# spcl/gemm_hls

Hardware: NVIDIA H100
Metric: GFLOP/s at N=16384 K=16384 M=16384 float (Multiply,Add) (higher is better)
Workload: dtype tf32 tensor-core multiply, f32 accumulate/storage

## Files before the change

gemm_hls_b200/csrc/gemm_tcgen05.cu:

```cuda
#include <cuda.h>
#include <cuda_fp16.h>
#include <cuda_runtime.h>

#include <algorithm>
#include <cstdlib>
#include <cstring>
#include <vector>

#include "common.cuh"
#include "fits_half.h"
#include "gemm_wgmma.cuh"
#include "ptx_sm90.cuh"
#include "tma_host.cuh"

namespace mm {
namespace {

__device__ __forceinline__ float round_tf32(float x) {
  uint32_t r;
  asm("cvt.rna.tf32.f32 %0, %1;" : "=r"(r) : "f"(x));
  const bool overflowed = (r & 0x7FFFFFFFu) == 0x7F800000u && (__float_as_uint(x) & 0x7FFFFFFFu) != 0x7F800000u;
  return __uint_as_float(overflowed ? ((r & 0x80000000u) | 0x7F7FE000u) : r);
}

// ... 14 lines not shown
    v.y = round_tf32(v.y);
    v.z = round_tf32(v.z);
    v.w = round_tf32(v.w);
    dst[i] = v;
  }
}

constexpr int FP_TILE = 64;
constexpr int FP_THREADS = 256;

struct FloatPrepOperand {
  const float *src = nullptr;
  float *dst = nullptr;
  __half *dst16 = nullptr;
  unsigned int *fits = nullptr;
  const unsigned int *partner = nullptr;
  uint32_t partner_stride = 0;
  const unsigned int *other = nullptr;
  uint32_t other_count = 0;
  unsigned char *pending = nullptr;
  uint32_t src_rows = 0, src_cols = 0, tiles_c = 0, items_per_copy = 0, items = 0;
  bool transpose = false;
  bool vec = false;
};
struct FloatPrepArgs {
  FloatPrepOperand op[2];
};

struct FloatItemSmem {
  float tile[FP_TILE][FP_TILE + 1];
  int settled;
};

__device__ __forceinline__ bool settled_now(const FloatPrepOperand &o, uint32_t copy) {
  const volatile unsigned int *own = o.fits;
  if (own[copy] == 0u) return true;
  const volatile unsigned int *partner = o.partner;
  return partner != nullptr && partner[copy * o.partner_stride] == 0u;
}

template <bool COMPLETE>
__device__ __forceinline__ void float_item(const FloatPrepOperand &o, uint32_t item, FloatItemSmem &sm) {
  const uint32_t t = threadIdx.x;
  const uint32_t copy = item / o.items_per_copy;
  const uint32_t tile_i = item - copy * o.items_per_copy;
  const uint32_t r0 = tile_i / o.tiles_c * FP_TILE, c0 = tile_i % o.tiles_c * FP_TILE;
  const size_t base = size_t(copy) * o.src_rows * o.src_cols;
  const float *src = o.src + base;
  float v[16];
  bool fit = true;
  if (!o.transpose) {
#pragma unroll
    for (int j = 0; j < 2; ++j) {
      const uint32_t q = t + FP_THREADS * j, r = r0 + q / 8, c = c0 + 8 * (q % 8);
      float4 x = make_float4(0.f, 0.f, 0.f, 0.f), y = x;
      if (r < o.src_rows && c < o.src_cols) {
        const float4 *p = reinterpret_cast<const float4 *>(src + size_t(r) * o.src_cols + c);
        x = p[0];
        y = p[1];
      }
      v[8 * j + 0] = x.x; v[8 * j + 1] = x.y; v[8 * j + 2] = x.z; v[8 * j + 3] = x.w;
      v[8 * j + 4] = y.x; v[8 * j + 5] = y.y; v[8 * j + 6] = y.z; v[8 * j + 7] = y.w;
    }
  } else {
#pragma unroll
    for (int j = 0; j < 4; ++j) {
      const uint32_t f = t + FP_THREADS * j, r = r0 + f / 16, c = c0 + 4 * (f % 16);
      float4 x = make_float4(0.f, 0.f, 0.f, 0.f);
      if (r < o.src_rows) {
        const float *p = src + size_t(r) * o.src_cols + c;
        if (o.vec) {
          if (c < o.src_cols) x = *reinterpret_cast<const float4 *>(p);
        } else {
          if (c + 0 < o.src_cols) x.x = p[0];
          if (c + 1 < o.src_cols) x.y = p[1];
          if (c + 2 < o.src_cols) x.z = p[2];
          if (c + 3 < o.src_cols) x.w = p[3];
        }
      }
      v[4 * j + 0] = x.x; v[4 * j + 1] = x.y; v[4 * j + 2] = x.z; v[4 * j + 3] = x.w;
    }
  }
#pragma unroll
  for (int e = 0; e < 16; ++e) {
    v[e] = round_tf32(v[e]);
    if (!COMPLETE) fit = fit && tf32_fits_half(__float_as_uint(v[e]));
  }
  if (o.transpose) {
#pragma unroll
    for (int j = 0; j < 4; ++j) {
      const uint32_t f = t + FP_THREADS * j, r = f / 16, c = 4 * (f % 16);
#pragma unroll
      for (int e = 0; e < 4; ++e) sm.tile[r][c + e] = v[4 * j + e];
    }
  }
  if (!COMPLETE && t == 0) sm.settled = settled_now(o, copy);
  __syncthreads();
  const bool settled = COMPLETE || sm.settled;
  float *dst = o.dst + base;
  __half *dst16 = o.dst16 + base;
  const uint32_t ld = o.transpose ? o.src_rows : o.src_cols;
  if (!o.transpose) {
#pragma unroll
    for (int j = 0; j < 2; ++j) {
      const uint32_t q = t + FP_THREADS * j, r = r0 + q / 8, c = c0 + 8 * (q % 8);
      if (r >= o.src_rows || c >= o.src_cols) continue;
      const size_t off = size_t(r) * ld + c;
      const float *w = v + 8 * j;
      if (settled) {
        reinterpret_cast<float4 *>(dst + off)[0] = make_float4(w[0], w[1], w[2], w[3]);
        reinterpret_cast<float4 *>(dst + off)[1] = make_float4(w[4], w[5], w[6], w[7]);
      } else {
        *reinterpret_cast<uint4 *>(dst16 + off) =
            make_uint4(half2_bits(w[0], w[1]), half2_bits(w[2], w[3]), half2_bits(w[4], w[5]), half2_bits(w[6], w[7]));
      }
    }
  } else if (settled) {
#pragma unroll
    for (int j = 0; j < 4; ++j) {
      const uint32_t idx = t + FP_THREADS * j, m = idx % 4 + 4 * (idx / 64), g = idx / 4 % 16;
      if (c0 + m >= o.src_cols || r0 + 4 * g >= o.src_rows) continue;
      float4 x;
      x.x = sm.tile[4 * g + 0][m];
      x.y = sm.tile[4 * g + 1][m];
      x.z = sm.tile[4 * g + 2][m];
      x.w = sm.tile[4 * g + 3][m];
      *reinterpret_cast<float4 *>(dst + size_t(c0 + m) * ld + r0 + 4 * g) = x;
    }
  } else {
#pragma unroll
// ... 436 lines not shown

int float_prep_grid(const void *kernel, uint32_t items) {
  MM_CUDA_TRY(cudaFuncSetAttribute(kernel, cudaFuncAttributePreferredSharedMemoryCarveout,
                                   cudaSharedmemCarveoutMaxShared));
  int per_sm = 0;
  MM_CUDA_TRY(cudaOccupancyMaxActiveBlocksPerMultiprocessor(&per_sm, kernel, FP_THREADS, 0));
  return int(std::max<uint32_t>(1u, std::min<uint32_t>(items, uint32_t(std::max(per_sm, 1) * num_sms()))));
}
}

int tcgen05_prepare_float(bool complete, const void *a, unsigned row0, unsigned rows, const void *b, unsigned n,
                          unsigned k, unsigned m, int flags, const Tuning &t, const GemmBatch &batch, void *scratch,
                          size_t scratch_bytes, cudaStream_t stream) {
  const HalfScratch hs = tcgen05_half_scratch(scratch, scratch_bytes, MM_DTYPE_FLOAT, n, k, m, flags, t, batch);
  if (hs.fits_a == nullptr) return fail(MM_ERR_INVALID, "tcgen05_prepare_float: float on the default datapath only");
  if (row0 % FP_TILE != 0) return fail(MM_ERR_INVALID, "tcgen05_prepare_float: A's first row must be a multiple of 64");
  unsigned char *sp = static_cast<unsigned char *>(scratch);
  const bool shared_a = batch.count > 1 && batch.shared_a, shared_b = batch.count > 1 && batch.shared_b;
  FloatPrepArgs args;
  if (b != nullptr) {
    FloatPrepOperand &o = args.op[0];
    o = float_operand(b, reinterpret_cast<float *>(sp), static_cast<__half *>(hs.b), k, m, batch.b_copies(), true,
                      hs.fits_b, hs.pending_b);
    o.partner = shared_b ? nullptr : hs.fits_a;
    o.partner_stride = shared_a ? 0 : 1;
    o.other = hs.fits_a;
    o.other_count = batch.a_copies();
  }
  if (a != nullptr) {
    const bool transposed = (flags & MM_FLAG_TRANSPOSED_A) != 0;
    if (transposed && (row0 != 0 || rows != n)) return fail(MM_ERR_INVALID, "A stored K x N is prepared whole");
    const size_t first = size_t(row0) * k;
    float *aprep = reinterpret_cast<float *>(sp + tcgen05_bt_bytes(MM_DTYPE_FLOAT, k, m, flags, t, batch.b_copies()));
    FloatPrepOperand &o = args.op[1];
    o = float_operand(a, aprep + first, static_cast<__half *>(hs.a) + first, transposed ? k : rows,
                      transposed ? rows : k, batch.a_copies(), transposed, hs.fits_a,
                      hs.pending_a + size_t(row0 / FP_TILE) * ceil_div(k, FP_TILE));
    o.partner = shared_a ? nullptr : hs.fits_b;
    o.partner_stride = shared_b ? 0 : 1;
    o.other = hs.fits_b;
    o.other_count = batch.b_copies();
  }
  const uint32_t items = args.op[0].items + args.op[1].items;
  if (complete) {
    const int grid = float_prep_grid(reinterpret_cast<const void *>(complete_tf32_kernel), items);
    complete_tf32_kernel<<<grid, FP_THREADS, 0, stream>>>(args);
// ... 135 lines not shown
```

gemm_hls_b200/csrc/gemm_wgmma.cuh:

```cuda
#pragma once

#include <cuda.h>
#include <cuda_bf16.h>
#include <cuda_fp16.h>
#include <cuda_runtime.h>

#include <algorithm>
#include <cstring>
#include <type_traits>

#include "common.cuh"
#include "ptx_sm90.cuh"
#include "tma_host.cuh"

namespace mm {
namespace {

constexpr int BLOCK_M = 128;
constexpr int BLOCK_K_BYTES = 128;
constexpr int WGMMA_K_BYTES = 32;
constexpr int NUM_THREADS = 384;
constexpr int CONSUMER_WARPS = 8;
constexpr int EPI_ROWS = 16;
constexpr int EPI_BUF_BYTES = 2048;
constexpr int EPI_BYTES = CONSUMER_WARPS * EPI_BUF_BYTES;
constexpr int BAR_BYTES = 256;
constexpr int MAX_DYN_SMEM = 232448;

template <int CG, int BN>
struct Geo {
  static constexpr int LOAD_N = BN / CG;
  static constexpr int A_STAGE_BYTES = BLOCK_M * BLOCK_K_BYTES;
  static constexpr int B_STAGE_BYTES = BN * BLOCK_K_BYTES;
  static constexpr int STAGE_BYTES = A_STAGE_BYTES + B_STAGE_BYTES;
  static constexpr int FIT = (MAX_DYN_SMEM - 1024 - BAR_BYTES - EPI_BYTES) / STAGE_BYTES;
  static constexpr int MAX_STAGES = FIT < 8 ? FIT : 8;
  static constexpr int TILE_ROWS = BLOCK_M * CG;
  static constexpr size_t smem_bytes(int stages) {
    return size_t(stages) * STAGE_BYTES + EPI_BYTES + 1024  + BAR_BYTES;
  }
};

struct TileCoord {
  uint32_t r, c;
  uint32_t prob;
};

__device__ __forceinline__ TileCoord tile_coord(uint32_t t, uint32_t tiles_r, uint32_t tiles_c,
// ... 179 lines not shown
        const int32_t a_row = tc.prob * p.a_prob_rows + tc.r * G::TILE_ROWS + cta_rank * BLOCK_M;
        const int32_t b_row = tc.prob * p.b_prob_rows + tc.c * BN + cta_rank * G::LOAD_N;
        if (p.b_ready != nullptr && int32_t(tc.c) != ready_panel) {
          const unsigned int *flag = p.b_ready + tc.c;
          const long long t0 = clock64();
          while (ld_acquire_gpu(flag) < p.b_ready_target) {
            if (clock64() - t0 > (1ll << 34)) __trap();
          }
          asm volatile("fence.proxy.async.global;" ::: "memory");
          ready_panel = int32_t(tc.c);
        }
        const bool h = half_tile(tc);
        const CUtensorMap *map_a = h ? &tmap_a16 : &tmap_a;
        const CUtensorMap *map_b = h ? &tmap_b16 : &tmap_b;
        const uint32_t tile_kb = h ? num_kb16 : num_kb;
        const int32_t kb_elems = h ? BLOCK_K_BYTES / 2 : BLOCK_K_ELEMS;
        for (uint32_t kb = 0; kb < tile_kb; ++kb) {
          ptx::mbar_wait(empty_bar(stage), phase ^ 1);
          const uint32_t sa = smem_a0 + stage * G::A_STAGE_BYTES;
          const uint32_t sb = smem_b0 + stage * G::B_STAGE_BYTES + cta_rank * G::LOAD_N * BLOCK_K_BYTES;
          const int32_t k0 = kb * kb_elems;
          ptx::mbar_arrive_expect_tx(full_bar(stage), G::STAGE_BYTES);
          ptx::tma_load_2d(sa, map_a, full_bar(stage), k0, a_row, p.l2_policy);
          if (CG == 1) {
            ptx::tma_load_2d(sb, map_b, full_bar(stage), k0, b_row, p.l2_policy);
          } else {
            ptx::tma_load_2d_multicast(sb, map_b, full_bar(stage), k0, b_row, 0x3, p.l2_policy);
          }
          if (++stage == STAGES) { stage = 0; phase ^= 1; }
        }
        if (p.tile_sync != nullptr && cta_rank == 0) atomicAdd(p.tile_sync, 1u);
      }
    }
  } else {
    ptx::setmaxnreg_inc<232>();
    const uint32_t wg = warp / 4 - 1;
    const uint32_t cwarp = warp - 4;
    const uint32_t buf = epi0 + cwarp * EPI_BUF_BYTES;
    const uint32_t peer = cta_rank ^ 1u;
    uint32_t stage = 0, phase = 0;
    uint32_t acc[BN / 2];
    for (uint32_t t = group_id; t < num_tiles; t += num_groups) {
      const TileCoord tc = tile_coord(t, tiles_r, tiles_c, p.raster_group);
      auto mainloop = [&](auto kind, uint32_t tile_kb) {
        uint32_t prev = 0;
        for (uint32_t kb = 0; kb < tile_kb; ++kb) {
          ptx::mbar_wait(full_bar(stage), phase);
          const uint64_t adesc = ptx::make_smem_desc_k_sw128(smem_a0 + stage * G::A_STAGE_BYTES + wg * 64 * BLOCK_K_BYTES);
          const uint64_t bdesc = ptx::make_smem_desc_k_sw128(smem_b0 + stage * G::B_STAGE_BYTES);
          ptx::wgmma_fence();
#pragma unroll
          for (int k = 0; k < BLOCK_K_BYTES / WGMMA_K_BYTES; ++k) {
            ptx::wgmma<decltype(kind)::value, BN>(acc, adesc + uint64_t(k * (WGMMA_K_BYTES >> 4)),
                                                  bdesc + uint64_t(k * (WGMMA_K_BYTES >> 4)),
                                                  (kb | uint32_t(k)) != 0u ? 1u : 0u);
          }
          ptx::wgmma_commit();
          ptx::wgmma_wait<1>();
          if (kb > 0 && lane == 0) {
            ptx::mbar_arrive(empty_bar(prev));
            if (CG == 2) ptx::mbar_arrive_cluster(empty_bar(prev), peer);
          }
          prev = stage;
          if (++stage == STAGES) { stage = 0; phase ^= 1; }
        }
        ptx::wgmma_wait<0>();
        if (lane == 0) {
          ptx::mbar_arrive(empty_bar(prev));
          if (CG == 2) ptx::mbar_arrive_cluster(empty_bar(prev), peer);
        }
      };
      if (KIND == ptx::KIND_TF32 && half_tile(tc)) {
        mainloop(std::integral_constant<int, ptx::KIND_F16>{}, num_kb16);
      } else {
        mainloop(std::integral_constant<int, KIND>{}, num_kb);
      }

      using P = Pair<TOut>;
      const uint32_t row0 = tc.r * G::TILE_ROWS + cta_rank * BLOCK_M + cwarp * EPI_ROWS;
      const uint32_t r_in = lane / 4, c_in = 2 * (lane % 4);
      if (p.tma_store) {
        constexpr uint32_t PITCH = 32 * sizeof(TOut);
        constexpr uint32_t SW_MASK = PITCH / 16 - 1;
#pragma unroll
        for (int chunk = 0; chunk < BN / 32; ++chunk) {
          const uint32_t col = tc.c * BN + chunk * 32;
          if (row0 < rows && col < cols) {
            typename P::T old[4][2];
            if constexpr (ACC) {
              const TOut *Cp = C + size_t(tc.prob) * rows * cols;
#pragma unroll
              for (int j = 0; j < 4; ++j) {
#pragma unroll
                for (int i = 0; i < 2; ++i) {
                  const uint32_t row = row0 + r_in + 8 * i, c = col + 8 * j + c_in;
                  old[j][i] = typename P::T{};
// ... 88 lines not shown
uint32_t elem_bytes(int dtype) { return dtype == MM_DTYPE_FLOAT ? 4u : (dtype == MM_DTYPE_UINT8 ? 1u : 2u); }

int encode(CUtensorMap *map, CUtensorMapDataType dt, const void *base, uint64_t inner, uint64_t outer, uint64_t pitch_bytes,
           uint32_t box_inner, uint32_t box_outer, CUtensorMapSwizzle swizzle, const char *what) {
  EncodeTiledFn enc = get_encode_fn();
  if (!enc) return fail(MM_ERR_CUDA, "cuTensorMapEncodeTiled entry point not available");
  cuuint64_t gdim[2] = {inner, outer};
  cuuint64_t gstride[1] = {pitch_bytes};
  cuuint32_t box[2] = {box_inner, box_outer};
  cuuint32_t estr[2] = {1, 1};
  CUresult r = enc(map, dt, 2, const_cast<void *>(base), gdim, gstride, box, estr, CU_TENSOR_MAP_INTERLEAVE_NONE,
                   swizzle, CU_TENSOR_MAP_L2_PROMOTION_L2_256B, CU_TENSOR_MAP_FLOAT_OOB_FILL_NONE);
  if (r != CUDA_SUCCESS) {
    return fail(MM_ERR_CUDA, std::string("cuTensorMapEncodeTiled (") + what + ") failed with CUresult " +
                                 std::to_string(int(r)));
  }
  return MM_OK;
}

int make_operand_map(CUtensorMap *map, const void *base, int dtype, uint64_t rows, uint64_t k_elems, uint32_t box_rows) {
  const uint32_t eb = elem_bytes(dtype);
  return encode(map, tma_dtype(dtype), base, k_elems, rows, k_elems * eb, uint32_t(BLOCK_K_BYTES / eb), box_rows,
                CU_TENSOR_MAP_SWIZZLE_128B, "K-major operand");
}

int make_c_map(CUtensorMap *map, void *base, int dtype, uint64_t rows, uint64_t m, uint64_t batch) {
  const uint32_t eb = elem_bytes(dtype);
  EncodeTiledFn enc = get_encode_fn();
  if (!enc) return fail(MM_ERR_CUDA, "cuTensorMapEncodeTiled entry point not available");
  cuuint64_t gdim[3] = {m, rows, batch};
  cuuint64_t gstride[2] = {m * eb, rows * m * eb};
  cuuint32_t box[3] = {32, EPI_ROWS, 1};
  cuuint32_t estr[3] = {1, 1, 1};
  const CUtensorMapSwizzle swizzle =
      eb == 4 ? CU_TENSOR_MAP_SWIZZLE_128B : (eb == 2 ? CU_TENSOR_MAP_SWIZZLE_64B : CU_TENSOR_MAP_SWIZZLE_32B);
  CUresult r = enc(map, tma_dtype(dtype), 3, base, gdim, gstride, box, estr, CU_TENSOR_MAP_INTERLEAVE_NONE, swizzle,
                   CU_TENSOR_MAP_L2_PROMOTION_L2_256B, CU_TENSOR_MAP_FLOAT_OOB_FILL_NONE);
  if (r != CUDA_SUCCESS) {
    return fail(MM_ERR_CUDA, "cuTensorMapEncodeTiled (C) failed with CUresult " + std::to_string(int(r)));
  }
  return MM_OK;
}

int num_sms() {
  int dev = 0, sms = 0;
  cudaGetDevice(&dev);
// ... 59 lines not shown
#undef MM_VARIANT
  return fail(MM_ERR_INVALID, "no wgmma kernel variant for this tuning (cta_group 1|2, block_n 128|256)");
}

int plan_gemm(int dtype, const void *a_op, const void *b_op, void *c, unsigned rows, unsigned k, unsigned m,
              const Tuning &t, unsigned int *tile_sync, const unsigned int *b_ready, unsigned b_ready_target,
              bool attributes_only, cudaStream_t stream, const GemmBatch &batch, const HalfOperands &half,
              CUtensorMap (&maps)[5], LaunchPlan *plan) {
  const size_t eb = elem_bytes(dtype);
  const int cg = t.cta_group(), bn = t.block_n();
  const bool use_half = dtype == MM_DTYPE_FLOAT && half.fits_a != nullptr;
  if (batch.count > 1 && b_ready != nullptr) return fail(MM_ERR_UNSUPPORTED, "batched calls need a complete B operand");
  std::memset(&maps[2], 0, sizeof(maps[2]));
  *plan = LaunchPlan{&maps[0], &maps[1], &maps[2], use_half ? &maps[3] : &maps[0], use_half ? &maps[4] : &maps[1],
                     c, {}, t.stages(), attributes_only, stream};
  if (!attributes_only) {
    int rc = make_operand_map(&maps[0], a_op, dtype, uint64_t(batch.a_copies()) * rows, k, BLOCK_M);
    if (rc != MM_OK) return rc;
    rc = make_operand_map(&maps[1], b_op, dtype, uint64_t(batch.b_copies()) * m, k, uint32_t(bn / cg));
    if (rc != MM_OK) return rc;
    if (use_half) {
      rc = make_operand_map(&maps[3], half.a, MM_DTYPE_HALF, uint64_t(batch.a_copies()) * rows, k, BLOCK_M);
      if (rc != MM_OK) return rc;
      rc = make_operand_map(&maps[4], half.b, MM_DTYPE_HALF, uint64_t(batch.b_copies()) * m, k, uint32_t(bn / cg));
      if (rc != MM_OK) return rc;
    }
    if (t.tma_store()) {
      rc = make_c_map(&maps[2], c, dtype, rows, m, batch.count);
      if (rc != MM_OK) return rc;
    }
  }
  GemmParams &p = plan->p;
  p.rows = rows;
  p.cols = m;
  p.batch = batch.count;
  p.a_prob_rows = batch.shared_a ? 0u : rows;
  p.b_prob_rows = batch.shared_b ? 0u : m;
  p.k_bytes = uint32_t(size_t(k) * eb);
  p.raster_group = uint32_t(std::max(1, t.raster_rows()));
  p.tma_store = t.tma_store() ? 1u : 0u;
  p.b_ready_target = b_ready_target;
  p.l2_policy = t.l2_policy() == 1 ? ptx::L2_EVICT_FIRST : (t.l2_policy() == 2 ? ptx::L2_EVICT_LAST : ptx::L2_EVICT_NORMAL);
  p.tile_sync = t.tile_sync() ? tile_sync : nullptr;
  p.b_ready = b_ready;
  p.fits_a = use_half ? half.fits_a : nullptr;
  p.fits_b = use_half ? half.fits_b : nullptr;
  return MM_OK;
// ... 15 lines not shown
```

gemm_hls_b200/csrc/ptx_sm90.cuh:

```cuda
#pragma once

#include <cuda_runtime.h>

#include <cstdint>

namespace mm {
namespace ptx {

__device__ __forceinline__ uint32_t smem_u32(const void *p) {
  return static_cast<uint32_t>(__cvta_generic_to_shared(p));
}

__device__ __forceinline__ uint32_t lane_id() {
  uint32_t l;
  asm volatile("mov.u32 %0, %%laneid;" : "=r"(l));
  return l;
}

__device__ __forceinline__ void mbar_init(uint32_t bar, uint32_t arrive_count) {
  asm volatile("mbarrier.init.shared::cta.b64 [%0], %1;" ::"r"(bar), "r"(arrive_count) : "memory");
}
__device__ __forceinline__ void fence_mbar_init() {
  asm volatile("fence.mbarrier_init.release.cluster;" ::: "memory");
}
// ... 44 lines not shown
__device__ __forceinline__ void tma_load_2d_multicast(uint32_t smem_dst, const void *tmap, uint32_t bar,
                                                      int32_t c0, int32_t c1, uint16_t cta_mask, uint64_t l2_policy) {
  asm volatile(
      "cp.async.bulk.tensor.2d.shared::cluster.global.mbarrier::complete_tx::bytes.multicast::cluster.L2::cache_hint"
      " [%0], [%1, {%4, %5}], [%2], %3, %6;" ::"r"(smem_dst),
      "l"(reinterpret_cast<uint64_t>(tmap)), "r"(bar), "h"(cta_mask), "r"(c0), "r"(c1), "l"(l2_policy)
      : "memory");
}
__device__ __forceinline__ void tma_store_2d(const void *tmap, uint32_t smem_src, int32_t c0,
                                             int32_t c1) {
  asm volatile("cp.async.bulk.tensor.2d.global.shared::cta.bulk_group [%0, {%2, %3}], [%1];" ::"l"(
                   reinterpret_cast<uint64_t>(tmap)),
               "r"(smem_src), "r"(c0), "r"(c1)
               : "memory");
}
__device__ __forceinline__ void tma_load_3d(uint32_t smem_dst, const void *tmap, uint32_t bar,
                                            int32_t c0, int32_t c1, int32_t c2, uint64_t l2_policy) {
  asm volatile(
      "cp.async.bulk.tensor.3d.shared::cluster.global.mbarrier::complete_tx::bytes.L2::cache_hint"
      " [%0], [%1, {%3, %4, %5}], [%2], %6;" ::"r"(smem_dst),
      "l"(reinterpret_cast<uint64_t>(tmap)), "r"(bar), "r"(c0), "r"(c1), "r"(c2), "l"(l2_policy)
      : "memory");
}
__device__ __forceinline__ void tma_store_3d(const void *tmap, uint32_t smem_src, int32_t c0, int32_t c1,
                                             int32_t c2) {
  asm volatile("cp.async.bulk.tensor.3d.global.shared::cta.bulk_group [%0, {%2, %3, %4}], [%1];" ::"l"(
                   reinterpret_cast<uint64_t>(tmap)),
               "r"(smem_src), "r"(c0), "r"(c1), "r"(c2)
               : "memory");
}
__device__ __forceinline__ void tma_store_commit() { asm volatile("cp.async.bulk.commit_group;" ::: "memory"); }
template <int N>
__device__ __forceinline__ void tma_store_wait_read() {
  asm volatile("cp.async.bulk.wait_group.read %0;" ::"n"(N) : "memory");
}
template <int N>
__device__ __forceinline__ void tma_store_wait_all() {
  asm volatile("cp.async.bulk.wait_group %0;" ::"n"(N) : "memory");
}
__device__ __forceinline__ void fence_proxy_async_smem() {
  asm volatile("fence.proxy.async.shared::cta;" ::: "memory");
}

__device__ __forceinline__ void st_shared_v4(uint32_t addr, uint32_t a, uint32_t b, uint32_t c, uint32_t d) {
  asm volatile("st.shared.v4.b32 [%0], {%1, %2, %3, %4};" ::"r"(addr), "r"(a), "r"(b), "r"(c), "r"(d) : "memory");
}

template <uint32_t N>
__device__ __forceinline__ void setmaxnreg_dec() {
  asm volatile("setmaxnreg.dec.sync.aligned.u32 %0;" ::"n"(N));
}
template <uint32_t N>
__device__ __forceinline__ void setmaxnreg_inc() {
  asm volatile("setmaxnreg.inc.sync.aligned.u32 %0;" ::"n"(N));
}

enum : int { KIND_F16 = 0, KIND_TF32 = 1, KIND_I8 = 2, KIND_BF16 = 3 };

__device__ __forceinline__ void wgmma_fence() { asm volatile("wgmma.fence.sync.aligned;" ::: "memory"); }
__device__ __forceinline__ void wgmma_commit() { asm volatile("wgmma.commit_group.sync.aligned;" ::: "memory"); }
template <int N>
__device__ __forceinline__ void wgmma_wait() {
  asm volatile("wgmma.wait_group.sync.aligned %0;" ::"n"(N) : "memory");
}

__device__ __forceinline__ uint64_t make_smem_desc_k_sw128(uint32_t smem_addr) {
  uint64_t d = 0;
  d |= static_cast<uint64_t>((smem_addr & 0x3FFFFu) >> 4);
  d |= static_cast<uint64_t>(1) << 16;
  d |= static_cast<uint64_t>(1024u >> 4) << 32;
  d |= static_cast<uint64_t>(1) << 62;
  return d;
}

template <int KIND, int N>
__device__ __forceinline__ void wgmma(uint32_t (&d)[N / 2], uint64_t desc_a, uint64_t desc_b, uint32_t accumulate);

template <>
__device__ __forceinline__ void wgmma<KIND_F16, 128>(uint32_t (&d)[64], uint64_t desc_a, uint64_t desc_b, uint32_t accumulate) {
  asm volatile(
      "{\n\t.reg .pred p;\n\tsetp.ne.b32 p, %66, 0;\n\t"
      "wgmma.mma_async.sync.aligned.m64n128k16.f32.f16.f16 {%0, %1, %2, %3, %4, %5, %6, %7, %8, %9, %10, %11, %12, %13, %14, %15, %16, %17, %18, %19, %20, %21, %22, %23, %24, %25, %26, %27, %28, %29, %30, %31, %32, %33, %34, %35, %36, %37, %38, %39, %40, %41, %42, %43, %44, %45, %46, %47, %48, %49, %50, %51, %52, %53, %54, %55, %56, %57, %58, %59, %60, %61, %62, %63}, %64, %65, p, 1, 1, 0, 0;\n\t}"
      : "+r"(d[0]), "+r"(d[1]), "+r"(d[2]), "+r"(d[3]), "+r"(d[4]), "+r"(d[5]), "+r"(d[6]), "+r"(d[7]), "+r"(d[8]), "+r"(d[9]), "+r"(d[10]), "+r"(d[11]), "+r"(d[12]), "+r"(d[13]), "+r"(d[14]), "+r"(d[15]), "+r"(d[16]), "+r"(d[17]), "+r"(d[18]), "+r"(d[19]), "+r"(d[20]), "+r"(d[21]), "+r"(d[22]), "+r"(d[23]), "+r"(d[24]), "+r"(d[25]), "+r"(d[26]), "+r"(d[27]), "+r"(d[28]), "+r"(d[29]), "+r"(d[30]), "+r"(d[31]), "+r"(d[32]), "+r"(d[33]), "+r"(d[34]), "+r"(d[35]), "+r"(d[36]), "+r"(d[37]), "+r"(d[38]), "+r"(d[39]), "+r"(d[40]), "+r"(d[41]), "+r"(d[42]), "+r"(d[43]), "+r"(d[44]), "+r"(d[45]), "+r"(d[46]), "+r"(d[47]), "+r"(d[48]), "+r"(d[49]), "+r"(d[50]), "+r"(d[51]), "+r"(d[52]), "+r"(d[53]), "+r"(d[54]), "+r"(d[55]), "+r"(d[56]), "+r"(d[57]), "+r"(d[58]), "+r"(d[59]), "+r"(d[60]), "+r"(d[61]), "+r"(d[62]), "+r"(d[63])
      : "l"(desc_a), "l"(desc_b), "r"(accumulate)
      : "memory");
}

template <>
__device__ __forceinline__ void wgmma<KIND_TF32, 128>(uint32_t (&d)[64], uint64_t desc_a, uint64_t desc_b, uint32_t accumulate) {
  asm volatile(
      "{\n\t.reg .pred p;\n\tsetp.ne.b32 p, %66, 0;\n\t"
      "wgmma.mma_async.sync.aligned.m64n128k8.f32.tf32.tf32 {%0, %1, %2, %3, %4, %5, %6, %7, %8, %9, %10, %11, %12, %13, %14, %15, %16, %17, %18, %19, %20, %21, %22, %23, %24, %25, %26, %27, %28, %29, %30, %31, %32, %33, %34, %35, %36, %37, %38, %39, %40, %41, %42, %43, %44, %45, %46, %47, %48, %49, %50, %51, %52, %53, %54, %55, %56, %57, %58, %59, %60, %61, %62, %63}, %64, %65, p, 1, 1;\n\t}"
      : "+r"(d[0]), "+r"(d[1]), "+r"(d[2]), "+r"(d[3]), "+r"(d[4]), "+r"(d[5]), "+r"(d[6]), "+r"(d[7]), "+r"(d[8]), "+r"(d[9]), "+r"(d[10]), "+r"(d[11]), "+r"(d[12]), "+r"(d[13]), "+r"(d[14]), "+r"(d[15]), "+r"(d[16]), "+r"(d[17]), "+r"(d[18]), "+r"(d[19]), "+r"(d[20]), "+r"(d[21]), "+r"(d[22]), "+r"(d[23]), "+r"(d[24]), "+r"(d[25]), "+r"(d[26]), "+r"(d[27]), "+r"(d[28]), "+r"(d[29]), "+r"(d[30]), "+r"(d[31]), "+r"(d[32]), "+r"(d[33]), "+r"(d[34]), "+r"(d[35]), "+r"(d[36]), "+r"(d[37]), "+r"(d[38]), "+r"(d[39]), "+r"(d[40]), "+r"(d[41]), "+r"(d[42]), "+r"(d[43]), "+r"(d[44]), "+r"(d[45]), "+r"(d[46]), "+r"(d[47]), "+r"(d[48]), "+r"(d[49]), "+r"(d[50]), "+r"(d[51]), "+r"(d[52]), "+r"(d[53]), "+r"(d[54]), "+r"(d[55]), "+r"(d[56]), "+r"(d[57]), "+r"(d[58]), "+r"(d[59]), "+r"(d[60]), "+r"(d[61]), "+r"(d[62]), "+r"(d[63])
      : "l"(desc_a), "l"(desc_b), "r"(accumulate)
      : "memory");
}

// ... 37 lines not shown
      : "memory");
}

template <>
__device__ __forceinline__ void wgmma<KIND_BF16, 128>(uint32_t (&d)[64], uint64_t desc_a, uint64_t desc_b, uint32_t accumulate) {
  asm volatile(
      "{\n\t.reg .pred p;\n\tsetp.ne.b32 p, %66, 0;\n\t"
      "wgmma.mma_async.sync.aligned.m64n128k16.f32.bf16.bf16 {%0, %1, %2, %3, %4, %5, %6, %7, %8, %9, %10, %11, %12, %13, %14, %15, %16, %17, %18, %19, %20, %21, %22, %23, %24, %25, %26, %27, %28, %29, %30, %31, %32, %33, %34, %35, %36, %37, %38, %39, %40, %41, %42, %43, %44, %45, %46, %47, %48, %49, %50, %51, %52, %53, %54, %55, %56, %57, %58, %59, %60, %61, %62, %63}, %64, %65, p, 1, 1, 0, 0;\n\t}"
      : "+r"(d[0]), "+r"(d[1]), "+r"(d[2]), "+r"(d[3]), "+r"(d[4]), "+r"(d[5]), "+r"(d[6]), "+r"(d[7]), "+r"(d[8]), "+r"(d[9]), "+r"(d[10]), "+r"(d[11]), "+r"(d[12]), "+r"(d[13]), "+r"(d[14]), "+r"(d[15]), "+r"(d[16]), "+r"(d[17]), "+r"(d[18]), "+r"(d[19]), "+r"(d[20]), "+r"(d[21]), "+r"(d[22]), "+r"(d[23]), "+r"(d[24]), "+r"(d[25]), "+r"(d[26]), "+r"(d[27]), "+r"(d[28]), "+r"(d[29]), "+r"(d[30]), "+r"(d[31]), "+r"(d[32]), "+r"(d[33]), "+r"(d[34]), "+r"(d[35]), "+r"(d[36]), "+r"(d[37]), "+r"(d[38]), "+r"(d[39]), "+r"(d[40]), "+r"(d[41]), "+r"(d[42]), "+r"(d[43]), "+r"(d[44]), "+r"(d[45]), "+r"(d[46]), "+r"(d[47]), "+r"(d[48]), "+r"(d[49]), "+r"(d[50]), "+r"(d[51]), "+r"(d[52]), "+r"(d[53]), "+r"(d[54]), "+r"(d[55]), "+r"(d[56]), "+r"(d[57]), "+r"(d[58]), "+r"(d[59]), "+r"(d[60]), "+r"(d[61]), "+r"(d[62]), "+r"(d[63])
      : "l"(desc_a), "l"(desc_b), "r"(accumulate)
      : "memory");
}

template <>
__device__ __forceinline__ void wgmma<KIND_BF16, 256>(uint32_t (&d)[128], uint64_t desc_a, uint64_t desc_b, uint32_t accumulate) {
  asm volatile(
      "{\n\t.reg .pred p;\n\tsetp.ne.b32 p, %130, 0;\n\t"
      "wgmma.mma_async.sync.aligned.m64n256k16.f32.bf16.bf16 {%0, %1, %2, %3, %4, %5, %6, %7, %8, %9, %10, %11, %12, %13, %14, %15, %16, %17, %18, %19, %20, %21, %22, %23, %24, %25, %26, %27, %28, %29, %30, %31, %32, %33, %34, %35, %36, %37, %38, %39, %40, %41, %42, %43, %44, %45, %46, %47, %48, %49, %50, %51, %52, %53, %54, %55, %56, %57, %58, %59, %60, %61, %62, %63, %64, %65, %66, %67, %68, %69, %70, %71, %72, %73, %74, %75, %76, %77, %78, %79, %80, %81, %82, %83, %84, %85, %86, %87, %88, %89, %90, %91, %92, %93, %94, %95, %96, %97, %98, %99, %100, %101, %102, %103, %104, %105, %106, %107, %108, %109, %110, %111, %112, %113, %114, %115, %116, %117, %118, %119, %120, %121, %122, %123, %124, %125, %126, %127}, %128, %129, p, 1, 1, 0, 0;\n\t}"
      : "+r"(d[0]), "+r"(d[1]), "+r"(d[2]), "+r"(d[3]), "+r"(d[4]), "+r"(d[5]), "+r"(d[6]), "+r"(d[7]), "+r"(d[8]), "+r"(d[9]), "+r"(d[10]), "+r"(d[11]), "+r"(d[12]), "+r"(d[13]), "+r"(d[14]), "+r"(d[15]), "+r"(d[16]), "+r"(d[17]), "+r"(d[18]), "+r"(d[19]), "+r"(d[20]), "+r"(d[21]), "+r"(d[22]), "+r"(d[23]), "+r"(d[24]), "+r"(d[25]), "+r"(d[26]), "+r"(d[27]), "+r"(d[28]), "+r"(d[29]), "+r"(d[30]), "+r"(d[31]), "+r"(d[32]), "+r"(d[33]), "+r"(d[34]), "+r"(d[35]), "+r"(d[36]), "+r"(d[37]), "+r"(d[38]), "+r"(d[39]), "+r"(d[40]), "+r"(d[41]), "+r"(d[42]), "+r"(d[43]), "+r"(d[44]), "+r"(d[45]), "+r"(d[46]), "+r"(d[47]), "+r"(d[48]), "+r"(d[49]), "+r"(d[50]), "+r"(d[51]), "+r"(d[52]), "+r"(d[53]), "+r"(d[54]), "+r"(d[55]), "+r"(d[56]), "+r"(d[57]), "+r"(d[58]), "+r"(d[59]), "+r"(d[60]), "+r"(d[61]), "+r"(d[62]), "+r"(d[63]), "+r"(d[64]), "+r"(d[65]), "+r"(d[66]), "+r"(d[67]), "+r"(d[68]), "+r"(d[69]), "+r"(d[70]), "+r"(d[71]), "+r"(d[72]), "+r"(d[73]), "+r"(d[74]), "+r"(d[75]), "+r"(d[76]), "+r"(d[77]), "+r"(d[78]), "+r"(d[79]), "+r"(d[80]), "+r"(d[81]), "+r"(d[82]), "+r"(d[83]), "+r"(d[84]), "+r"(d[85]), "+r"(d[86]), "+r"(d[87]), "+r"(d[88]), "+r"(d[89]), "+r"(d[90]), "+r"(d[91]), "+r"(d[92]), "+r"(d[93]), "+r"(d[94]), "+r"(d[95]), "+r"(d[96]), "+r"(d[97]), "+r"(d[98]), "+r"(d[99]), "+r"(d[100]), "+r"(d[101]), "+r"(d[102]), "+r"(d[103]), "+r"(d[104]), "+r"(d[105]), "+r"(d[106]), "+r"(d[107]), "+r"(d[108]), "+r"(d[109]), "+r"(d[110]), "+r"(d[111]), "+r"(d[112]), "+r"(d[113]), "+r"(d[114]), "+r"(d[115]), "+r"(d[116]), "+r"(d[117]), "+r"(d[118]), "+r"(d[119]), "+r"(d[120]), "+r"(d[121]), "+r"(d[122]), "+r"(d[123]), "+r"(d[124]), "+r"(d[125]), "+r"(d[126]), "+r"(d[127])
      : "l"(desc_a), "l"(desc_b), "r"(accumulate)
      : "memory");
}

}
}
```

Measured before the change: 672,500.

## Keep half-precision B in MN-major layout and load it with 3D TMA boxes

For the tf32 path, B operand tiles whose values fit in fp16 are now written in their original (non-transposed) row-major layout during preparation. This skips the shared-memory transpose in the prep kernel for the half case. The GEMM mainloop then loads B with 3D TMA boxes of 64 columns and uses an MN-major smem descriptor with the transpose bit set on the f16 wgmma. The added descriptor, tensor-map and wgmma variants must all agree on the swizzle and stride layout to produce correct results.

```diff
diff --git a/gemm_hls_b200/csrc/gemm_tcgen05.cu b/gemm_hls_b200/csrc/gemm_tcgen05.cu
--- a/gemm_hls_b200/csrc/gemm_tcgen05.cu
+++ b/gemm_hls_b200/csrc/gemm_tcgen05.cu
@@ -60,6 +60,7 @@
   uint32_t src_rows = 0, src_cols = 0, tiles_c = 0, items_per_copy = 0, items = 0;
   bool transpose = false;
   bool vec = false;
+  bool flat16 = false;
 };
 struct FloatPrepArgs {
   FloatPrepOperand op[2];
@@ -85,9 +86,11 @@
   const uint32_t r0 = tile_i / o.tiles_c * FP_TILE, c0 = tile_i % o.tiles_c * FP_TILE;
   const size_t base = size_t(copy) * o.src_rows * o.src_cols;
   const float *src = o.src + base;
+  const bool flat_loads = !o.transpose || o.flat16;
+  const bool tile_early = o.transpose && (COMPLETE || !o.flat16);
   float v[16];
   bool fit = true;
-  if (!o.transpose) {
+  if (flat_loads) {
 #pragma unroll
     for (int j = 0; j < 2; ++j) {
       const uint32_t q = t + FP_THREADS * j, r = r0 + q / 8, c = c0 + 8 * (q % 8);
@@ -124,26 +127,40 @@
     v[e] = round_tf32(v[e]);
     if (!COMPLETE) fit = fit && tf32_fits_half(__float_as_uint(v[e]));
   }
-  if (o.transpose) {
-#pragma unroll
-    for (int j = 0; j < 4; ++j) {
-      const uint32_t f = t + FP_THREADS * j, r = f / 16, c = 4 * (f % 16);
-#pragma unroll
-      for (int e = 0; e < 4; ++e) sm.tile[r][c + e] = v[4 * j + e];
-    }
-  }
+  auto fill_tile = [&] {
+    if (flat_loads) {
+#pragma unroll
+      for (int j = 0; j < 2; ++j) {
+        const uint32_t q = t + FP_THREADS * j, r = q / 8, c = 8 * (q % 8);
+#pragma unroll
+        for (int e = 0; e < 8; ++e) sm.tile[r][c + e] = v[8 * j + e];
+      }
+    } else {
+#pragma unroll
+      for (int j = 0; j < 4; ++j) {
+        const uint32_t f = t + FP_THREADS * j, r = f / 16, c = 4 * (f % 16);
+#pragma unroll
+        for (int e = 0; e < 4; ++e) sm.tile[r][c + e] = v[4 * j + e];
+      }
+    }
+  };
+  if (tile_early) fill_tile();
   if (!COMPLETE && t == 0) sm.settled = settled_now(o, copy);
   __syncthreads();
   const bool settled = COMPLETE || sm.settled;
+  if (!COMPLETE && o.flat16 && settled) {
+    fill_tile();
+    __syncthreads();
+  }
   float *dst = o.dst + base;
   __half *dst16 = o.dst16 + base;
   const uint32_t ld = o.transpose ? o.src_rows : o.src_cols;
-  if (!o.transpose) {
+  if (!o.transpose || (o.flat16 && !settled)) {
 #pragma unroll
     for (int j = 0; j < 2; ++j) {
       const uint32_t q = t + FP_THREADS * j, r = r0 + q / 8, c = c0 + 8 * (q % 8);
       if (r >= o.src_rows || c >= o.src_cols) continue;
-      const size_t off = size_t(r) * ld + c;
+      const size_t off = size_t(r) * o.src_cols + c;
       const float *w = v + 8 * j;
       if (settled) {
         reinterpret_cast<float4 *>(dst + off)[0] = make_float4(w[0], w[1], w[2], w[3]);
@@ -626,6 +643,7 @@
     FloatPrepOperand &o = args.op[0];
     o = float_operand(b, reinterpret_cast<float *>(sp), static_cast<__half *>(hs.b), k, m, batch.b_copies(), true,
                       hs.fits_b, hs.pending_b);
+    o.flat16 = true;
     o.partner = shared_b ? nullptr : hs.fits_a;
     o.partner_stride = shared_a ? 0 : 1;
     o.other = hs.fits_a;
diff --git a/gemm_hls_b200/csrc/gemm_wgmma.cuh b/gemm_hls_b200/csrc/gemm_wgmma.cuh
--- a/gemm_hls_b200/csrc/gemm_wgmma.cuh
+++ b/gemm_hls_b200/csrc/gemm_wgmma.cuh
@@ -24,6 +24,8 @@
 constexpr int EPI_ROWS = 16;
 constexpr int EPI_BUF_BYTES = 2048;
 constexpr int EPI_BYTES = CONSUMER_WARPS * EPI_BUF_BYTES;
+constexpr int MN_BOX = 64;
+constexpr int MN_BOX_BYTES = MN_BOX * BLOCK_K_BYTES;
 constexpr int BAR_BYTES = 256;
 constexpr int MAX_DYN_SMEM = 232448;
 
@@ -249,7 +251,18 @@
           const int32_t k0 = kb * kb_elems;
           ptx::mbar_arrive_expect_tx(full_bar(stage), G::STAGE_BYTES);
           ptx::tma_load_2d(sa, map_a, full_bar(stage), k0, a_row, p.l2_policy);
-          if (CG == 1) {
+          if (KIND == ptx::KIND_TF32 && h) {
+            const int32_t n0 = tc.c * BN + cta_rank * G::LOAD_N, b_prob = p.b_prob_rows ? int32_t(tc.prob) : 0;
+#pragma unroll
+            for (int j = 0; j < G::LOAD_N / MN_BOX; ++j) {
+              if (CG == 1) {
+                ptx::tma_load_3d(sb + j * MN_BOX_BYTES, map_b, full_bar(stage), n0 + j * MN_BOX, k0, b_prob, p.l2_policy);
+              } else {
+                ptx::tma_load_3d_multicast(sb + j * MN_BOX_BYTES, map_b, full_bar(stage), n0 + j * MN_BOX, k0, b_prob,
+                                           0x3, p.l2_policy);
+              }
+            }
+          } else if (CG == 1) {
             ptx::tma_load_2d(sb, map_b, full_bar(stage), k0, b_row, p.l2_policy);
           } else {
             ptx::tma_load_2d_multicast(sb, map_b, full_bar(stage), k0, b_row, 0x3, p.l2_policy);
@@ -270,16 +283,19 @@
     for (uint32_t t = group_id; t < num_tiles; t += num_groups) {
       const TileCoord tc = tile_coord(t, tiles_r, tiles_c, p.raster_group);
       auto mainloop = [&](auto kind, uint32_t tile_kb) {
+        constexpr bool MN_B = decltype(kind)::value == ptx::KIND_F16_MN_B;
+        constexpr uint32_t B_STEP = MN_B ? (WGMMA_K_BYTES / 2) * BLOCK_K_BYTES : WGMMA_K_BYTES;
         uint32_t prev = 0;
         for (uint32_t kb = 0; kb < tile_kb; ++kb) {
           ptx::mbar_wait(full_bar(stage), phase);
           const uint64_t adesc = ptx::make_smem_desc_k_sw128(smem_a0 + stage * G::A_STAGE_BYTES + wg * 64 * BLOCK_K_BYTES);
-          const uint64_t bdesc = ptx::make_smem_desc_k_sw128(smem_b0 + stage * G::B_STAGE_BYTES);
+          const uint64_t bdesc = MN_B ? ptx::make_smem_desc_mn_sw128(smem_b0 + stage * G::B_STAGE_BYTES, MN_BOX_BYTES)
+                                      : ptx::make_smem_desc_k_sw128(smem_b0 + stage * G::B_STAGE_BYTES);
           ptx::wgmma_fence();
 #pragma unroll
           for (int k = 0; k < BLOCK_K_BYTES / WGMMA_K_BYTES; ++k) {
             ptx::wgmma<decltype(kind)::value, BN>(acc, adesc + uint64_t(k * (WGMMA_K_BYTES >> 4)),
-                                                  bdesc + uint64_t(k * (WGMMA_K_BYTES >> 4)),
+                                                  bdesc + uint64_t(k * (B_STEP >> 4)),
                                                   (kb | uint32_t(k)) != 0u ? 1u : 0u);
           }
           ptx::wgmma_commit();
@@ -298,7 +314,7 @@
         }
       };
       if (KIND == ptx::KIND_TF32 && half_tile(tc)) {
-        mainloop(std::integral_constant<int, ptx::KIND_F16>{}, num_kb16);
+        mainloop(std::integral_constant<int, ptx::KIND_F16_MN_B>{}, num_kb16);
       } else {
         mainloop(std::integral_constant<int, KIND>{}, num_kb);
       }
@@ -433,6 +449,22 @@
   const uint32_t eb = elem_bytes(dtype);
   return encode(map, tma_dtype(dtype), base, k_elems, rows, k_elems * eb, uint32_t(BLOCK_K_BYTES / eb), box_rows,
                 CU_TENSOR_MAP_SWIZZLE_128B, "K-major operand");
+}
+
+int make_half_b_map(CUtensorMap *map, const void *base, uint64_t k, uint64_t m, uint64_t copies) {
+  EncodeTiledFn enc = get_encode_fn();
+  if (!enc) return fail(MM_ERR_CUDA, "cuTensorMapEncodeTiled entry point not available");
+  cuuint64_t gdim[3] = {m, k, copies};
+  cuuint64_t gstride[2] = {m * 2, k * m * 2};
+  cuuint32_t box[3] = {MN_BOX, BLOCK_K_BYTES / 2, 1};
+  cuuint32_t estr[3] = {1, 1, 1};
+  CUresult r = enc(map, CU_TENSOR_MAP_DATA_TYPE_FLOAT16, 3, const_cast<void *>(base), gdim, gstride, box, estr,
+                   CU_TENSOR_MAP_INTERLEAVE_NONE, CU_TENSOR_MAP_SWIZZLE_128B, CU_TENSOR_MAP_L2_PROMOTION_L2_256B,
+                   CU_TENSOR_MAP_FLOAT_OOB_FILL_NONE);
+  if (r != CUDA_SUCCESS) {
+    return fail(MM_ERR_CUDA, "cuTensorMapEncodeTiled (fp16 B) failed with CUresult " + std::to_string(int(r)));
+  }
+  return MM_OK;
 }
 
 int make_c_map(CUtensorMap *map, void *base, int dtype, uint64_t rows, uint64_t m, uint64_t batch) {
@@ -538,7 +570,7 @@
     if (use_half) {
       rc = make_operand_map(&maps[3], half.a, MM_DTYPE_HALF, uint64_t(batch.a_copies()) * rows, k, BLOCK_M);
       if (rc != MM_OK) return rc;
-      rc = make_operand_map(&maps[4], half.b, MM_DTYPE_HALF, uint64_t(batch.b_copies()) * m, k, uint32_t(bn / cg));
+      rc = make_half_b_map(&maps[4], half.b, k, m, batch.b_copies());
       if (rc != MM_OK) return rc;
     }
     if (t.tma_store()) {
diff --git a/gemm_hls_b200/csrc/ptx_sm90.cuh b/gemm_hls_b200/csrc/ptx_sm90.cuh
--- a/gemm_hls_b200/csrc/ptx_sm90.cuh
+++ b/gemm_hls_b200/csrc/ptx_sm90.cuh
@@ -90,6 +90,14 @@
       "l"(reinterpret_cast<uint64_t>(tmap)), "r"(bar), "r"(c0), "r"(c1), "r"(c2), "l"(l2_policy)
       : "memory");
 }
+__device__ __forceinline__ void tma_load_3d_multicast(uint32_t smem_dst, const void *tmap, uint32_t bar, int32_t c0,
+                                                      int32_t c1, int32_t c2, uint16_t cta_mask, uint64_t l2_policy) {
+  asm volatile(
+      "cp.async.bulk.tensor.3d.shared::cluster.global.mbarrier::complete_tx::bytes.multicast::cluster.L2::cache_hint"
+      " [%0], [%1, {%4, %5, %6}], [%2], %3, %7;" ::"r"(smem_dst),
+      "l"(reinterpret_cast<uint64_t>(tmap)), "r"(bar), "h"(cta_mask), "r"(c0), "r"(c1), "r"(c2), "l"(l2_policy)
+      : "memory");
+}
 __device__ __forceinline__ void tma_store_3d(const void *tmap, uint32_t smem_src, int32_t c0, int32_t c1,
                                              int32_t c2) {
   asm volatile("cp.async.bulk.tensor.3d.global.shared::cta.bulk_group [%0, {%2, %3, %4}], [%1];" ::"l"(
@@ -123,7 +131,7 @@
   asm volatile("setmaxnreg.inc.sync.aligned.u32 %0;" ::"n"(N));
 }
 
-enum : int { KIND_F16 = 0, KIND_TF32 = 1, KIND_I8 = 2, KIND_BF16 = 3 };
+enum : int { KIND_F16 = 0, KIND_TF32 = 1, KIND_I8 = 2, KIND_BF16 = 3, KIND_F16_MN_B = 4 };
 
 __device__ __forceinline__ void wgmma_fence() { asm volatile("wgmma.fence.sync.aligned;" ::: "memory"); }
 __device__ __forceinline__ void wgmma_commit() { asm volatile("wgmma.commit_group.sync.aligned;" ::: "memory"); }
@@ -141,6 +149,15 @@
   return d;
 }
 
+__device__ __forceinline__ uint64_t make_smem_desc_mn_sw128(uint32_t smem_addr, uint32_t mn_atom_bytes) {
+  uint64_t d = 0;
+  d |= static_cast<uint64_t>((smem_addr & 0x3FFFFu) >> 4);
+  d |= static_cast<uint64_t>(mn_atom_bytes >> 4) << 16;
+  d |= static_cast<uint64_t>(1024u >> 4) << 32;
+  d |= static_cast<uint64_t>(1) << 62;
+  return d;
+}
+
 template <int KIND, int N>
 __device__ __forceinline__ void wgmma(uint32_t (&d)[N / 2], uint64_t desc_a, uint64_t desc_b, uint32_t accumulate);
 
@@ -224,5 +241,25 @@
       : "memory");
 }
 
-}
-}
+template <>
+__device__ __forceinline__ void wgmma<KIND_F16_MN_B, 128>(uint32_t (&d)[64], uint64_t desc_a, uint64_t desc_b, uint32_t accumulate) {
+  asm volatile(
+      "{\n\t.reg .pred p;\n\tsetp.ne.b32 p, %66, 0;\n\t"
+      "wgmma.mma_async.sync.aligned.m64n128k16.f32.f16.f16 {%0, %1, %2, %3, %4, %5, %6, %7, %8, %9, %10, %11, %12, %13, %14, %15, %16, %17, %18, %19, %20, %21, %22, %23, %24, %25, %26, %27, %28, %29, %30, %31, %32, %33, %34, %35, %36, %37, %38, %39, %40, %41, %42, %43, %44, %45, %46, %47, %48, %49, %50, %51, %52, %53, %54, %55, %56, %57, %58, %59, %60, %61, %62, %63}, %64, %65, p, 1, 1, 0, 1;\n\t}"
+      : "+r"(d[0]), "+r"(d[1]), "+r"(d[2]), "+r"(d[3]), "+r"(d[4]), "+r"(d[5]), "+r"(d[6]), "+r"(d[7]), "+r"(d[8]), "+r"(d[9]), "+r"(d[10]), "+r"(d[11]), "+r"(d[12]), "+r"(d[13]), "+r"(d[14]), "+r"(d[15]), "+r"(d[16]), "+r"(d[17]), "+r"(d[18]), "+r"(d[19]), "+r"(d[20]), "+r"(d[21]), "+r"(d[22]), "+r"(d[23]), "+r"(d[24]), "+r"(d[25]), "+r"(d[26]), "+r"(d[27]), "+r"(d[28]), "+r"(d[29]), "+r"(d[30]), "+r"(d[31]), "+r"(d[32]), "+r"(d[33]), "+r"(d[34]), "+r"(d[35]), "+r"(d[36]), "+r"(d[37]), "+r"(d[38]), "+r"(d[39]), "+r"(d[40]), "+r"(d[41]), "+r"(d[42]), "+r"(d[43]), "+r"(d[44]), "+r"(d[45]), "+r"(d[46]), "+r"(d[47]), "+r"(d[48]), "+r"(d[49]), "+r"(d[50]), "+r"(d[51]), "+r"(d[52]), "+r"(d[53]), "+r"(d[54]), "+r"(d[55]), "+r"(d[56]), "+r"(d[57]), "+r"(d[58]), "+r"(d[59]), "+r"(d[60]), "+r"(d[61]), "+r"(d[62]), "+r"(d[63])
+      : "l"(desc_a), "l"(desc_b), "r"(accumulate)
+      : "memory");
+}
+
+template <>
+__device__ __forceinline__ void wgmma<KIND_F16_MN_B, 256>(uint32_t (&d)[128], uint64_t desc_a, uint64_t desc_b, uint32_t accumulate) {
+  asm volatile(
+      "{\n\t.reg .pred p;\n\tsetp.ne.b32 p, %130, 0;\n\t"
+      "wgmma.mma_async.sync.aligned.m64n256k16.f32.f16.f16 {%0, %1, %2, %3, %4, %5, %6, %7, %8, %9, %10, %11, %12, %13, %14, %15, %16, %17, %18, %19, %20, %21, %22, %23, %24, %25, %26, %27, %28, %29, %30, %31, %32, %33, %34, %35, %36, %37, %38, %39, %40, %41, %42, %43, %44, %45, %46, %47, %48, %49, %50, %51, %52, %53, %54, %55, %56, %57, %58, %59, %60, %61, %62, %63, %64, %65, %66, %67, %68, %69, %70, %71, %72, %73, %74, %75, %76, %77, %78, %79, %80, %81, %82, %83, %84, %85, %86, %87, %88, %89, %90, %91, %92, %93, %94, %95, %96, %97, %98, %99, %100, %101, %102, %103, %104, %105, %106, %107, %108, %109, %110, %111, %112, %113, %114, %115, %116, %117, %118, %119, %120, %121, %122, %123, %124, %125, %126, %127}, %128, %129, p, 1, 1, 0, 1;\n\t}"
+      : "+r"(d[0]), "+r"(d[1]), "+r"(d[2]), "+r"(d[3]), "+r"(d[4]), "+r"(d[5]), "+r"(d[6]), "+r"(d[7]), "+r"(d[8]), "+r"(d[9]), "+r"(d[10]), "+r"(d[11]), "+r"(d[12]), "+r"(d[13]), "+r"(d[14]), "+r"(d[15]), "+r"(d[16]), "+r"(d[17]), "+r"(d[18]), "+r"(d[19]), "+r"(d[20]), "+r"(d[21]), "+r"(d[22]), "+r"(d[23]), "+r"(d[24]), "+r"(d[25]), "+r"(d[26]), "+r"(d[27]), "+r"(d[28]), "+r"(d[29]), "+r"(d[30]), "+r"(d[31]), "+r"(d[32]), "+r"(d[33]), "+r"(d[34]), "+r"(d[35]), "+r"(d[36]), "+r"(d[37]), "+r"(d[38]), "+r"(d[39]), "+r"(d[40]), "+r"(d[41]), "+r"(d[42]), "+r"(d[43]), "+r"(d[44]), "+r"(d[45]), "+r"(d[46]), "+r"(d[47]), "+r"(d[48]), "+r"(d[49]), "+r"(d[50]), "+r"(d[51]), "+r"(d[52]), "+r"(d[53]), "+r"(d[54]), "+r"(d[55]), "+r"(d[56]), "+r"(d[57]), "+r"(d[58]), "+r"(d[59]), "+r"(d[60]), "+r"(d[61]), "+r"(d[62]), "+r"(d[63]), "+r"(d[64]), "+r"(d[65]), "+r"(d[66]), "+r"(d[67]), "+r"(d[68]), "+r"(d[69]), "+r"(d[70]), "+r"(d[71]), "+r"(d[72]), "+r"(d[73]), "+r"(d[74]), "+r"(d[75]), "+r"(d[76]), "+r"(d[77]), "+r"(d[78]), "+r"(d[79]), "+r"(d[80]), "+r"(d[81]), "+r"(d[82]), "+r"(d[83]), "+r"(d[84]), "+r"(d[85]), "+r"(d[86]), "+r"(d[87]), "+r"(d[88]), "+r"(d[89]), "+r"(d[90]), "+r"(d[91]), "+r"(d[92]), "+r"(d[93]), "+r"(d[94]), "+r"(d[95]), "+r"(d[96]), "+r"(d[97]), "+r"(d[98]), "+r"(d[99]), "+r"(d[100]), "+r"(d[101]), "+r"(d[102]), "+r"(d[103]), "+r"(d[104]), "+r"(d[105]), "+r"(d[106]), "+r"(d[107]), "+r"(d[108]), "+r"(d[109]), "+r"(d[110]), "+r"(d[111]), "+r"(d[112]), "+r"(d[113]), "+r"(d[114]), "+r"(d[115]), "+r"(d[116]), "+r"(d[117]), "+r"(d[118]), "+r"(d[119]), "+r"(d[120]), "+r"(d[121]), "+r"(d[122]), "+r"(d[123]), "+r"(d[124]), "+r"(d[125]), "+r"(d[126]), "+r"(d[127])
+      : "l"(desc_a), "l"(desc_b), "r"(accumulate)
+      : "memory");
+}
+
+}
+}
```

Result: no change. 671,500 (median of 6 runs) (-0.1%).
